# Tom94/practical-path-guiding

Hardware: NVIDIA H100
Metric: Msamples/sec (paths x bounces) (higher is better)
Workload: dtype f32

## Files before the change

### practical-path-guiding_b200/csrc/ppg_bounce.cuh

```cuda
#pragma once
#include "ppg_wavefront.cuh"

namespace ppg {

template <bool FIRST, int RECORD, bool NEE, bool SMEM, bool FULL>
__global__ void __launch_bounds__(SMEM ? PPG_BOUNCE_BLOCK : PPG_BOUNCE_BLOCK_HBM, SMEM ? PPG_MIN_BLOCKS : PPG_MIN_BLOCKS_HBM) bounce_kernel(const __grid_constant__ RenderParams P) {
    const SceneAccess<SMEM> sc(P.scene);
    sc.stage();
    const uint32_t nIn = FIRST ? P.nPaths : *P.liveIn;
    uint32_t raysLocal = 0, recLocal = 0, levelsLocal = 0;
    __shared__ uint32_t binStart[PPG_BINS + 1];
    const bool binned = !SMEM && P.order != nullptr;
    if (binned) {
        if (threadIdx.x == 0) { uint32_t acc = 0; for (uint32_t b = 0; b < PPG_BINS; ++b) { binStart[b] = acc; acc += P.binCount[b]; } binStart[PPG_BINS] = acc; }
        __syncthreads();
    }

    const uint32_t lane = threadIdx.x & 31u;
    uint32_t claimBase = 0, claimLeft = 0;
    for (;;) {
        if (claimLeft == 0) {
            if (lane == 0) claimBase = atomicAdd(P.work, 32u * PPG_CLAIM);
            claimBase = __shfl_sync(0xffffffffu, claimBase, 0);
            claimLeft = PPG_CLAIM;
        }
        if (claimBase >= nIn) break;
        uint32_t i = claimBase + lane;
        claimBase += 32u; --claimLeft;
        bool alive = i < nIn;
        if (binned && alive) {
            uint32_t b = 0;
            while (b + 1 < PPG_BINS && i >= binStart[b + 1]) ++b;
            i = __ldg(&P.order[(size_t) b * P.binStride + (i - binStart[b])]);
        }
        float3 o, d, thr, Li; float eta = 1.f, rrRecip = 1.f, mint, maxt;
        float prevWoPdf = 0.f; float3 prevRefN = f3(0, 0, 0); uint32_t prevSlot = 0;
        uint32_t pathId = 0, nVertices = 0, flags = 0;
        Pcg32 rng; rng.state = 0; rng.inc = 1;
        if (alive) {
            if (FIRST) {
                pathId = i;
                uint64_t sampleIndex;
                camera_ray(P, i, rng, sampleIndex, o, d, mint, maxt);
                thr = f3(1, 1, 1); Li = f3(0, 0, 0);
            } else {
                const float4 a = __ldcs(&P.in.s0[i]), b = __ldcs(&P.in.s1[i]), c = __ldcs(&P.in.s2[i]), e = __ldcs(&P.in.s3[i]), f = __ldcs(&P.in.s4[i]);
                o = f3(a.x, a.y, a.z); d = f3(a.w, b.x, b.y); thr = f3(b.z, b.w, c.x); eta = c.y; Li = f3(c.z, c.w, e.x);
                pathId = __float_as_uint(e.y);
                rng.state = ((uint64_t) __float_as_uint(e.w) << 32) | __float_as_uint(e.z);
                const uint64_t sampleIndex = ((uint64_t) __float_as_uint(f.y) << 32) | __float_as_uint(f.x);
                rng.inc = (sampleIndex << 1) | 1u;
                const uint32_t nf = __float_as_uint(f.z); nVertices = nf & 0xffu; flags = nf >> 8;
                rrRecip = f.w;
                if (NEE) { const float4 g5 = __ldcs(&P.in.s5[i]), g6 = __ldcs(&P.in.s6[i]); prevWoPdf = g5.x; prevRefN = f3(g5.y, g5.z, g5.w); prevSlot = __float_as_uint(g6.x); }
                mint = surface_ray_mint(o);
                maxt = __int_as_float(0x7f800000);
            }
        }
        bool wroteVertex = false, wroteNee = false, unscattered = FIRST;
        Hit hit; bool rayOk = false, found = false;
        if (alive) {
            ++raysLocal;
            rayOk = isfinite(o.x + o.y + o.z) && isfinite(d.x + d.y + d.z);
            if (!rayOk) atomicAdd(&P.counters[5], 1ull);
            if (!SMEM && P.hits) {
                const float4 hv = __ldcs(&P.hits[i]);
                const uint32_t w = __float_as_uint(hv.w);
                hit.t = hv.x; hit.u = hv.y; hit.v = hv.z; hit.tri = 0; hit.prim = w;
                found = rayOk && w != 0xFFFFFFFFu;
                if (found && !(w & PPG_SPHERE_BIT)) { hit.tri = w; hit.prim = __float_as_uint(sc.accel(3 * w + 2).z); }
                if (!found) { hit.t = __int_as_float(0x7f800000); hit.prim = 0xFFFFFFFFu; }
            } else
                found = rayOk && bvh_intersect<FULL>(sc, o, d, mint, maxt, hit);
        }
        __syncwarp();
        if (alive) {
            bool cont = found;
            if (FULL && !found && rayOk && P.scene.envW) {
                const bool viaNull = !FIRST && (flags & PPG_FLAG_NULL);
                const bool add = (FIRST || viaNull) ? ((FIRST || (flags & PPG_FLAG_UNSCATTERED)) && !P.hideEmitters) : true;
                if (add) {
                    float3 Lenv = thr * env_eval(P.scene, d);
                    if (NEE && !FIRST && !viaNull && P.doNee && !(prevSlot >> 31))
                        Lenv = Lenv * mi_weight(prevWoPdf, pdf_emitter_direct<FULL>(P.scene, PPG_ENV_EMITTER, o, prevRefN, d, f3(0, 0, 0), 0.f));
                    Li = Li + Lenv;
                }
                if (NEE && !FIRST && !viaNull && P.training && P.neeMode == 2 && ((prevSlot >> 30) & 1u)) {
                    const uint32_t ps = prevSlot & 0x3fffffffu;
                    float4 pv = P.prevSlab.v2[ps]; pv.x = Li.x; pv.y = Li.y; pv.z = Li.z; P.prevSlab.v2[ps] = pv;
                }
            }
            Its its;
            if (cont) {
                fill_its<FULL>(sc, hit, o, d, its);
                float3 Lhit = f3(0, 0, 0);
                const bool viaNull = FULL && !FIRST && (flags & PPG_FLAG_NULL);
                unscattered = FIRST || (FULL && (flags & PPG_FLAG_UNSCATTERED));
                if (FULL && viaNull) {
                    if (its.emitter >= 0 && unscattered && !P.hideEmitters && dot(its.shN, -d) > 0.f) {
                        const float4 r = sc.radiance(its.emitter);
                        Li = Li + thr * f3(r.x, r.y, r.z);
                    }
                } else if (FULL && !FIRST && its.emitter < 0 && bsdf_has_null(load_bsdf<FULL>(sc, its.bsdf))) {
                    int qEmitter; float3 qN; float qDist;
                    const float3 value = look_through(sc, o, d, its, hit.t, P.maxDepth - P.depth, qEmitter, qN, qDist);
                    if (!is_zero(value)) {
                        Lhit = thr * value;
                        if (NEE && P.doNee && !(prevSlot >> 31)) Lhit = Lhit * mi_weight(prevWoPdf, pdf_emitter_direct<FULL>(sc.g, qEmitter, o, prevRefN, d, qN, qDist));
                        Li = Li + Lhit;
                    }
                } else if (its.emitter >= 0 && (!FIRST || !P.hideEmitters)) {
                    if (dot(its.shN, -d) > 0.f) {
                        const float4 r = sc.radiance(its.emitter);
                        Lhit = thr * f3(r.x, r.y, r.z);
                        if (NEE && !FIRST && P.doNee && !(prevSlot >> 31)) {
                            const float emitterPdf = pdf_emitter_direct<FULL>(sc.g, its.emitter, o, prevRefN, d, its.shN, hit.t);
                            Lhit = Lhit * mi_weight(prevWoPdf, emitterPdf);
                        }
                        Li = Li + Lhit;
                    }
                }
                if (NEE && !FIRST && P.training && P.neeMode == 2 && ((prevSlot >> 30) & 1u)) {
                    const uint32_t ps = prevSlot & 0x3fffffffu;
                    float4 pv = P.prevSlab.v2[ps]; pv.x = Li.x; pv.y = Li.y; pv.z = Li.z; P.prevSlab.v2[ps] = pv;
                }
                thr = thr * rrRecip;
                if (flags & PPG_FLAG_DYING) cont = false;
                if (P.depth >= P.maxDepth && P.maxDepth != -1) cont = false;
            }
            if (cont) {
                const float wiDotGeoN = -dot(its.geoN, d);
                if (wiDotGeoN * its.wi.z < 0.f && P.strictNormals) cont = false;
            }
            if (cont) {
                Bsdf bsdf = load_bsdf<FULL>(sc, its.bsdf);
                const float3 n0 = its.shN;
                const bool bump = FULL && bsdf.bumpTex && !(hit.prim & PPG_SPHERE_BIT);
                if (FULL && (bsdf.reflTex | bsdf.bumpTex) && !(hit.prim & PPG_SPHERE_BIT)) apply_textures(sc, hit, d, its, bsdf);
                const bool smooth = bsdf_has_smooth(bsdf);
                int levels = 0; uint32_t leaf = 0; float4 la = make_float4(0, 0, 0, 0);
                if (smooth) {
                    leaf = stree_lookup(P.tree.snodes, P.tree.stable, P.tree.aabbMin, P.tree.extent, its.p, levels);
                    la = __ldg(&P.tree.leafA[leaf]);
                }
                float frac = P.fixedFraction;
                if (smooth && P.lossMode != 0) frac = logistic(la.z);
                float woPdf, bsdfPdf, dTreePdf, bsEta = 1.f; float3 wo, bsdfWeight; bool isDelta = false, isNull = false;
                float sx = rng.next1D(); const float sy = rng.next1D();
                if (!P.isBuilt || !smooth) {
                    bsdfWeight = bsdf_sample(bsdf, its.wi, sx, sy, wo, bsEta, isDelta, bsdfPdf, rng, isNull);
                    if (bump && !is_zero(bsdfWeight) && dot(its.toWorld(wo), n0) * wo.z <= 0.f) bsdfWeight = f3(0, 0, 0);
                    woPdf = bsdfPdf; dTreePdf = 0.f;
                } else {
                    const SampNode *tree = P.tree.samp + __float_as_uint(la.x);
                    const bool valid = __float_as_uint(la.w) & 1u;
                    float3 result; bool zero = false, deltaEarly = false;
                    if (sx < frac) {
                        sx /= frac;
                        result = bsdf_sample(bsdf, its.wi, sx, sy, wo, bsEta, isDelta, bsdfPdf, rng, isNull);
                        if (bump && !is_zero(result) && dot(its.toWorld(wo), n0) * wo.z <= 0.f) result = f3(0, 0, 0);
                        if (is_zero(result)) { woPdf = bsdfPdf = dTreePdf = 0.f; zero = true; }
                        else if (FULL && isDelta) { dTreePdf = 0.f; woPdf = bsdfPdf * frac; result = result * (1.0f / frac); deltaEarly = true; }
                        else result = result * bsdfPdf;
                    } else {
                        const float2 c2 = dtree_sample(tree, valid, rng);
                        const float3 dw = canonical_to_dir(c2);
                        wo = its.toLocal(dw);
                        result = (bump && dot(dw, n0) * wo.z <= 0.f) ? f3(0, 0, 0) : bsdf_eval(bsdf, its.wi, wo);
                    }
                    if (zero) bsdfWeight = f3(0, 0, 0);
                    else if (deltaEarly) bsdfWeight = result;
                    else {
                        bsdfPdf = (bump && dot(its.toWorld(wo), n0) * wo.z <= 0.f) ? 0.0f : bsdf_pdf(bsdf, its.wi, wo);
                        if (!isfinite(bsdfPdf)) { woPdf = 0.f; dTreePdf = 0.f; }
                        else {
                            dTreePdf = dtree_pdf(tree, valid, dir_to_canonical(its.toWorld(wo)));
                            woPdf = frac * bsdfPdf + (1.f - frac) * dTreePdf;
                        }
                        bsdfWeight = (woPdf == 0.f) ? f3(0, 0, 0) : result * (1.0f / woPdf);
                    }
                }
                const float3 refN = bsdf_has_transmission_or_backside(bsdf) ? f3(0, 0, 0) : n0;
                if (NEE && P.doNee && smooth) {
                    const float ex = rng.next1D(), ey = rng.next1D();
                    DirectSample ds; float dist;
                    if (sample_emitter_direct<FULL>(sc, its.p, refN, ex, ey, ds, dist)) {
                        const float smint = PPG_EPSILON * fmaxf(fmaxf(fabsf(its.p.x), fabsf(its.p.y)), fabsf(its.p.z));
                        Hit sh;
                        bool visible;
                        if (FULL) {
                            const float3 T = eval_transmittance(sc, its.p, ds.d, dist, P.maxDepth - P.depth - 1);
                            ds.value = ds.value * T; visible = !is_zero(ds.value);
                        } else visible = !bvh_intersect<FULL>(sc, its.p, ds.d, smint, dist * (1.f - PPG_SHADOW_EPSILON), sh);
                        if (visible) {
                            const float3 dl = its.toLocal(ds.d);
                            const float dlZ0 = bump ? dot(ds.d, n0) : dl.z;
                            if (!P.strictNormals || dot(its.geoN, ds.d) * dlZ0 > 0.f) {
                                const bool bumpReject = bump && dlZ0 * dl.z <= 0.f;
                                const float3 bsdfVal = bumpReject ? f3(0, 0, 0) : bsdf_eval(bsdf, its.wi, dl);
                                float nWoPdf = 0.f, nBsdfPdf = bumpReject ? 0.0f : bsdf_pdf(bsdf, its.wi, dl), nDTreePdf = 0.f;
                                if (!P.isBuilt) nWoPdf = nBsdfPdf;
                                else if (isfinite(nBsdfPdf)) {
                                    nDTreePdf = dtree_pdf(P.tree.samp + __float_as_uint(la.x), __float_as_uint(la.w) & 1u, dir_to_canonical(ds.d));
                                    nWoPdf = frac * nBsdfPdf + (1.f - frac) * nDTreePdf;
                                }
                                const float3 L = thr * (ds.value * bsdfVal) * mi_weight(ds.pdf, nWoPdf);
                                if (RECORD && P.neeMode != 2) {
                                    const float3 tv = thr * bsdfVal * (1.0f / ds.pdf);
                                    __stcs(&P.neeSlab.v0[i], make_float4(ds.d.x, ds.d.y, ds.d.z, ds.pdf));
                                    __stcs(&P.neeSlab.v1[i], make_float4(tv.x, tv.y, tv.z, __uint_as_float(leaf)));
                                    __stcs(&P.neeSlab.v2[i], make_float4(L.x, L.y, L.z, __uint_as_float(pathId | 0x40000000u)));
                                    __stcs(&P.neeSlab.v3[i], make_float4(bsdfVal.x, bsdfVal.y, bsdfVal.z, nBsdfPdf));
                                    __stcs(&P.neeSlab.v4[i], make_float4(its.p.x, its.p.y, its.p.z, nDTreePdf));
                                    __stcs(&P.neeSlab.v5[i], make_float4(__uint_as_float((uint32_t) (rng.inc >> 1)), __uint_as_float((uint32_t) (rng.inc >> 33)),
                                                                  __uint_as_float((uint32_t) levels | ((32u + (uint32_t) P.depth) << 8)), 0.f));
                                    wroteNee = true;
                                }
                                Li = Li + L;
                            }
                        }
                    }
                }
                if (is_zero(bsdfWeight)) cont = false;
                float3 woW = f3(0, 0, 0);
                if (cont) {
                    woW = its.toWorld(wo);
                    if (dot(its.geoN, woW) * (bump ? dot(woW, n0) : wo.z) <= 0.f && P.strictNormals) cont = false;
                }
                if (cont) {
                    o = its.p; d = woW;
                    thr = thr * bsdfWeight; eta *= bsEta;
                    if (RECORD && smooth && (!isDelta || P.lossMode != 0) && nVertices < PPG_MAX_VERTICES && (1.f / woPdf > 0.f)) {
                        __stcs(&P.slab.v0[i], make_float4(d.x, d.y, d.z, woPdf));
                        __stcs(&P.slab.v1[i], make_float4(thr.x, thr.y, thr.z, __uint_as_float(leaf)));
                        __stcs(&P.slab.v2[i], make_float4(Li.x, Li.y, Li.z, __uint_as_float(pathId | (isDelta ? 0x80000000u : 0u))));
                        if (RECORD == 2) {
                            const float3 bv = bsdfWeight * woPdf;
                            __stcs(&P.slab.v3[i], make_float4(bv.x, bv.y, bv.z, bsdfPdf));
                            __stcs(&P.slab.v4[i], make_float4(o.x, o.y, o.z, dTreePdf));
                            __stcs(&P.slab.v5[i], make_float4(__uint_as_float((uint32_t) (rng.inc >> 1)), __uint_as_float((uint32_t) (rng.inc >> 33)),
                                                       __uint_as_float((uint32_t) levels | (nVertices << 8)), 0.f));
                        }
                        wroteVertex = true; ++nVertices; ++recLocal; levelsLocal += levels;
                    }
                    if (NEE) { prevWoPdf = woPdf; prevRefN = refN; prevSlot = i | (isDelta ? 0x80000000u : 0u) | ((wroteVertex && !(FULL && isNull)) ? 0x40000000u : 0u); }
                    rrRecip = 1.f; flags = 0;
                    if (FULL && isNull) flags = PPG_FLAG_NULL | (unscattered ? PPG_FLAG_UNSCATTERED : 0u);
                    else if (P.depth >= P.rrDepth) {
                        float successProb = 1.0f;
                        if (smooth && !isDelta) {
                            if (!P.isBuilt) successProb = max3(thr) * eta * eta;
                            successProb = fmaxf(0.1f, fminf(successProb, 0.99f));
                        }
                        if (rng.next1D() >= successProb) flags |= PPG_FLAG_DYING;
                        else rrRecip = 1.0f / successProb;
                    }
                }
            }
            if (!cont) {
                __stcs(&P.liFinal[pathId], make_float4(Li.x, Li.y, Li.z, 1.f));
                alive = false;
            }
        }
        if (RECORD && i < nIn && !wroteVertex) __stcs(&P.slab.v2[i], make_float4(0.f, 0.f, 0.f, __uint_as_float(PPG_INVALID)));
        if (NEE && RECORD && P.neeMode != 2 && i < nIn && !wroteNee) __stcs(&P.neeSlab.v2[i], make_float4(0.f, 0.f, 0.f, __uint_as_float(PPG_INVALID)));
        const uint32_t slot = warp_compact(alive, P.liveOut);
        if (alive) {
            __stcs(&P.out.s0[slot], make_float4(o.x, o.y, o.z, d.x));
            __stcs(&P.out.s1[slot], make_float4(d.y, d.z, thr.x, thr.y));
            __stcs(&P.out.s2[slot], make_float4(thr.z, eta, Li.x, Li.y));
            __stcs(&P.out.s3[slot], make_float4(Li.z, __uint_as_float(pathId), __uint_as_float((uint32_t) rng.state), __uint_as_float((uint32_t) (rng.state >> 32))));
            __stcs(&P.out.s4[slot], make_float4(__uint_as_float((uint32_t) (rng.inc >> 1)), __uint_as_float((uint32_t) (rng.inc >> 33)),
                                         __uint_as_float(nVertices | (flags << 8)), rrRecip));
            if (NEE) {
                __stcs(&P.out.s5[slot], make_float4(prevWoPdf, prevRefN.x, prevRefN.y, prevRefN.z));
                __stcs(&P.out.s6[slot], make_float4(__uint_as_float(prevSlot), 0.f, 0.f, 0.f));
            }
        }
    }
    unsigned long long rays = raysLocal, rec = recLocal, lev = levelsLocal;
    for (int off = 16; off; off >>= 1) {
        rays += __shfl_xor_sync(0xffffffffu, rays, off);
        rec += __shfl_xor_sync(0xffffffffu, rec, off);
        lev += __shfl_xor_sync(0xffffffffu, lev, off);
    }
    if ((threadIdx.x & 31) == 0) {
        if (rays) atomicAdd(&P.counters[0], rays);
        if (rec) { atomicAdd(&P.counters[1], rec); atomicAdd(&P.counters[2], lev); }
    }
}

}
```

### practical-path-guiding_b200/csrc/ppg_device.cuh

```cuda
#pragma once
#include <cuda_runtime.h>
#include <cuda_fp16.h>
#include <stdint.h>
#include "ppg_scene_layout.h"

namespace ppg {

#define PPG_PI 3.14159265358979323846f
#define PPG_INV_PI 0.31830988618379067154f
#define PPG_EPSILON 1e-4f

__device__ __forceinline__ float3 f3(float x, float y, float z) { return make_float3(x, y, z); }
__device__ __forceinline__ float3 operator+(float3 a, float3 b) { return f3(a.x + b.x, a.y + b.y, a.z + b.z); }
__device__ __forceinline__ float3 operator-(float3 a, float3 b) { return f3(a.x - b.x, a.y - b.y, a.z - b.z); }
__device__ __forceinline__ float3 operator*(float3 a, float s) { return f3(a.x * s, a.y * s, a.z * s); }
__device__ __forceinline__ float3 operator*(float3 a, float3 b) { return f3(a.x * b.x, a.y * b.y, a.z * b.z); }
__device__ __forceinline__ float3 operator-(float3 a) { return f3(-a.x, -a.y, -a.z); }
__device__ __forceinline__ float dot(float3 a, float3 b) { return a.x * b.x + a.y * b.y + a.z * b.z; }
__device__ __forceinline__ float3 cross(float3 a, float3 b) { return f3(a.y * b.z - a.z * b.y, a.z * b.x - a.x * b.z, a.x * b.y - a.y * b.x); }
__device__ __forceinline__ float3 normalize(float3 a) { return a * (1.0f / sqrtf(dot(a, a))); }
__device__ __forceinline__ bool is_zero(float3 a) { return a.x == 0.f && a.y == 0.f && a.z == 0.f; }
__device__ __forceinline__ bool is_valid(float3 a) {
    return isfinite(a.x) && isfinite(a.y) && isfinite(a.z) && a.x >= 0.f && a.y >= 0.f && a.z >= 0.f;
}
// ... 33 lines not shown
__device__ __forceinline__ void seed_vertex_rng(Pcg32 &r, uint64_t seed, uint64_t sampleIndex, uint32_t ordinal) {
    r.seed(splitmix64((seed + 0x5851F42D4C957F2Dull) ^ splitmix64(sampleIndex * 64 + ordinal)), sampleIndex * 64 + ordinal);
}

#define PPG_ENV_EMITTER (-2)

struct Hit { float t, u, v; uint32_t tri; uint32_t prim; };

extern __shared__ float4 ppg_scene_smem[];
template <bool SMEM> struct SceneAccess {
    static constexpr bool kStaged = SMEM;
    const SceneView &g;
    uint32_t oGeom, oMeta, oBvh, oBsdf, oRadiance, oGroups;
    __device__ __forceinline__ SceneAccess(const SceneView &v) : g(v) {
        oGeom = 3 * v.nTris; oMeta = oGeom + 6 * v.nTris; oBvh = oMeta + v.nTris; oBsdf = oBvh + 2 * v.nBvhNodes;
        oRadiance = oBsdf + PPG_BSDF_F4 * v.nBsdfs; oGroups = oRadiance + v.nEmitters;
    }
    __device__ __forceinline__ float4 accel(uint32_t i) const { return SMEM ? ppg_scene_smem[i] : __ldg(&g.accel[i]); }
    __device__ __forceinline__ float4 geom(uint32_t i) const { return SMEM ? ppg_scene_smem[oGeom + i] : __ldg(&g.geom[i]); }
    __device__ __forceinline__ int4 meta(uint32_t i) const {
        if (SMEM) { const float4 m = ppg_scene_smem[oMeta + i]; return make_int4(__float_as_int(m.x), __float_as_int(m.y), __float_as_int(m.z), __float_as_int(m.w)); }
        return __ldg(&g.meta[i]);
    }
    __device__ __forceinline__ float4 bvh(uint32_t i) const { return SMEM ? ppg_scene_smem[oBvh + i] : __ldg(&g.bvh[i]); }
    __device__ __forceinline__ float4 bsdf(uint32_t i) const { return SMEM ? ppg_scene_smem[oBsdf + i] : __ldg(&g.bsdf[i]); }
    __device__ __forceinline__ float4 radiance(uint32_t i) const { return SMEM ? ppg_scene_smem[oRadiance + i] : __ldg(&g.radiance[i]); }
    __device__ __forceinline__ float4 groups(uint32_t i) const { return SMEM ? ppg_scene_smem[oGroups + i] : __ldg(&g.groups[i]); }
    __device__ __forceinline__ void stage() const {
        if (!SMEM) return;
        auto copy = [&](uint32_t off, const float4 *src, uint32_t n) { for (uint32_t i = threadIdx.x; i < n; i += blockDim.x) ppg_scene_smem[off + i] = src[i]; };
        copy(0, g.accel, 3 * g.nTris); copy(oGeom, g.geom, 6 * g.nTris); copy(oMeta, reinterpret_cast<const float4 *>(g.meta), g.nTris);
        copy(oBvh, g.bvh, 2 * g.nBvhNodes); copy(oBsdf, g.bsdf, PPG_BSDF_F4 * g.nBsdfs); copy(oRadiance, g.radiance, g.nEmitters); copy(oGroups, g.groups, 2 * g.nGroups);
        __syncthreads();
    }
};

__device__ __forceinline__ bool tri_intersect(const float4 A, const float4 B, const float4 C, float3 o, float3 d, float mint, float maxt,
                                              float &u, float &v, float &t) {
    const int k = __float_as_int(A.w);
    float o_u, o_v, o_k, d_u, d_v, d_k;
    if (k == 0) { o_u = o.y; o_v = o.z; o_k = o.x; d_u = d.y; d_v = d.z; d_k = d.x; }
    else if (k == 1) { o_u = o.z; o_v = o.x; o_k = o.y; d_u = d.z; d_v = d.x; d_k = d.y; }
    else if (k == 2) { o_u = o.x; o_v = o.y; o_k = o.z; d_u = d.x; d_v = d.y; d_k = d.z; }
    else return false;
    t = (A.z - o_u * A.x - o_v * A.y - o_k) / (d_u * A.x + d_v * A.y + d_k);
    if (!(t >= mint && t <= maxt)) return false;
    const float hu = o_u + t * d_u - B.x;
    const float hv = o_v + t * d_v - B.y;
    u = hv * B.z + hu * B.w;
    v = hu * C.x + hv * C.y;
    return u >= 0.f && v >= 0.f && u + v <= 1.0f;
}

template <class Acc>
__device__ __forceinline__ void tri_group_exact(const Acc &A_, uint32_t q, float o_u, float o_v, float o_k, float d_u, float d_v, float d_k,
                                                float mint, float maxt, Hit &hit) {
    const uint32_t fc = __float_as_uint(A_.groups(2 * q).w), last = (fc & 0xffffu) + (fc >> 16);
    for (uint32_t i = fc & 0xffffu; i < last; ++i) {
        const float4 A = A_.accel(3 * i), B = A_.accel(3 * i + 1), C = A_.accel(3 * i + 2);
        const float t = (A.z - o_u * A.x - o_v * A.y - o_k) / (d_u * A.x + d_v * A.y + d_k);
        if (t >= mint && t <= maxt) {
            const float hu = o_u + t * d_u - B.x, hv = o_v + t * d_v - B.y;
            const float u = hv * B.z + hu * B.w, v = hu * C.x + hv * C.y;
            if (u >= 0.f && v >= 0.f && u + v <= 1.0f) {
                const uint32_t prim = __float_as_uint(C.z);
                if (t < hit.t || (t == hit.t && prim < hit.prim)) { hit.t = t; hit.u = u; hit.v = v; hit.prim = prim; hit.tri = i; }
            }
        }
    }
}

__device__ __forceinline__ bool sphere_intersect(float4 cr, float3 ro, float3 rd, float mint, float maxt, float &t) {
    const double ox = (double) ro.x - (double) cr.x, oy = (double) ro.y - (double) cr.y, oz = (double) ro.z - (double) cr.z;
    const double dx = rd.x, dy = rd.y, dz = rd.z;
    const double A = __dadd_rn(__dadd_rn(__dmul_rn(dx, dx), __dmul_rn(dy, dy)), __dmul_rn(dz, dz));
    const double B = __dmul_rn(2.0, __dadd_rn(__dadd_rn(__dmul_rn(ox, dx), __dmul_rn(oy, dy)), __dmul_rn(oz, dz)));
    const double C = __dsub_rn(__dadd_rn(__dadd_rn(__dmul_rn(ox, ox), __dmul_rn(oy, oy)), __dmul_rn(oz, oz)), (double) (cr.w * cr.w));
    double nearT, farT;
    if (A == 0.0) { if (B != 0.0) nearT = farT = -C / B; else return false; }
    else {
        const double discrim = __dsub_rn(__dmul_rn(B, B), __dmul_rn(__dmul_rn(4.0, A), C));
        if (discrim < 0.0) return false;
        const double sqrtDiscrim = sqrt(discrim);
        const double temp = B < 0.0 ? __dmul_rn(-0.5, __dsub_rn(B, sqrtDiscrim)) : __dmul_rn(-0.5, __dadd_rn(B, sqrtDiscrim));
        nearT = temp / A; farT = C / temp;
        if (nearT > farT) { const double s = nearT; nearT = farT; farT = s; }
    }
    if (!(nearT <= (double) maxt && farT >= (double) mint)) return false;
    if (nearT < (double) mint) { if (farT > (double) maxt) return false; t = (float) farT; }
    else t = (float) nearT;
    return true;
}
__device__ __forceinline__ bool bvh_slab(float3 o, float3 inv, float mint, float tmax, const float4 n0, const float4 n1, float &tEntry) {
    float ta = (n0.x - o.x) * inv.x, tb = (n1.x - o.x) * inv.x; if (ta > tb) { const float s_ = ta; ta = tb; tb = s_; }
    float nearMax = fmaxf(__int_as_float(0xff800000), ta), farMin = fminf(__int_as_float(0x7f800000), tb);
    ta = (n0.y - o.y) * inv.y; tb = (n1.y - o.y) * inv.y; if (ta > tb) { const float s_ = ta; ta = tb; tb = s_; }
    nearMax = fmaxf(nearMax, ta); farMin = fminf(farMin, tb);
    ta = (n0.z - o.z) * inv.z; tb = (n1.z - o.z) * inv.z; if (ta > tb) { const float s_ = ta; ta = tb; tb = s_; }
    nearMax = fmaxf(nearMax, ta); farMin = fminf(farMin, tb);
    const float t0 = fmaxf(mint, nearMax * (nearMax > 0.f ? 1.0f - 1e-6f : 1.0f + 1e-6f)), t1 = fminf(tmax, farMin * (farMin > 0.f ? 1.0f + 1e-6f : 1.0f - 1e-6f));
    tEntry = t0;
    return t0 <= t1;
}
static __device__ __noinline__ Hit bvh_walk(const float4 *__restrict__ accel, const float4 *__restrict__ bvh, float3 o, float3 d, float mint, float maxt) {
    Hit hit; hit.t = __int_as_float(0x7f800000); hit.u = hit.v = 0.f; hit.prim = 0xFFFFFFFFu; hit.tri = 0;
    const float3 inv = f3(1.0f / d.x, 1.0f / d.y, 1.0f / d.z);
    auto slab = [&](const float4 n0, const float4 n1, float &tEntry) -> bool { return bvh_slab(o, inv, mint, fminf(maxt, hit.t), n0, n1, tEntry); };
    auto node = [&](uint32_t i) { return __ldg(&bvh[i]); };
    auto tri = [&](uint32_t i) { return __ldg(&accel[i]); };
    uint32_t stackN[PPG_BVH_STACK]; float stackT[PPG_BVH_STACK]; int sp = 0;
    uint32_t left, count;
    {
        const float4 r0 = node(0), r1 = node(1);
        float te;
        if (!slab(r0, r1, te)) return hit;
        left = __float_as_uint(r0.w); count = __float_as_uint(r1.w);
    }
    auto pop = [&]() -> bool {
        while (sp > 0) {
            --sp;
            if (stackT[sp] <= hit.t) { left = stackN[sp] & 0x0fffffffu; count = stackN[sp] >> 28; return true; }
        }
        return false;
    };
    bool done = false;
    for (;;) {
        while (count == 0u && !done) {
            const float4 a0 = node(2 * left), a1 = node(2 * left + 1), b0 = node(2 * left + 2), b1 = node(2 * left + 3);
            float ta, tb;
            const bool ha = slab(a0, a1, ta), hb = slab(b0, b1, tb);
            if (ha && hb) {
                const bool aFirst = ta <= tb;
                const float4 f0 = aFirst ? b0 : a0, f1 = aFirst ? b1 : a1, n0 = aFirst ? a0 : b0, n1 = aFirst ? a1 : b1;
                stackN[sp] = __float_as_uint(f0.w) | (__float_as_uint(f1.w) << 28); stackT[sp] = aFirst ? tb : ta; ++sp;
                left = __float_as_uint(n0.w); count = __float_as_uint(n1.w);
            } else if (ha) { left = __float_as_uint(a0.w); count = __float_as_uint(a1.w); }
            else if (hb) { left = __float_as_uint(b0.w); count = __float_as_uint(b1.w); }
            else done = !pop();
        }
        if (done) break;
        for (uint32_t i = left; i < left + count; ++i) {
            const float4 A = tri(3 * i), B = tri(3 * i + 1), C = tri(3 * i + 2);
            float u, v, t;
            if (tri_intersect(A, B, C, o, d, mint, maxt, u, v, t)) {
                const uint32_t prim = __float_as_uint(C.z);
                if (t < hit.t || (t == hit.t && prim < hit.prim)) { hit.t = t; hit.u = u; hit.v = v; hit.prim = prim; hit.tri = i; }
            }
        }
        if (!pop()) break;
    }
    return hit;
}
template <class Acc> __device__ __forceinline__ bool tri_scene_intersect(const Acc &A_, float3 o, float3 d, float mint, float maxt, Hit &hit);

template <bool SPHERES, class Acc>
__device__ __forceinline__ bool bvh_intersect(const Acc &A_, float3 o, float3 d, float mint, float maxt, Hit &hit) {
    bool found = tri_scene_intersect(A_, o, d, mint, maxt, hit);
    if (!SPHERES) return found;
    const SceneView &sc = A_.g;
    for (uint32_t k = 0; k < sc.nSpheres; ++k) {
        float t;
        if (sphere_intersect(__ldg(&sc.spheres[2 * k]), o, d, mint, maxt, t) && t < hit.t) { hit.t = t; hit.u = hit.v = 0.f; hit.prim = PPG_SPHERE_BIT | k; hit.tri = 0; found = true; }
    }
    return found;
}
template <class Acc>
__device__ __forceinline__ bool tri_scene_intersect(const Acc &A_, float3 o, float3 d, float mint, float maxt, Hit &hit) {
    const SceneView &sc = A_.g;
    hit.t = __int_as_float(0x7f800000); hit.prim = 0xFFFFFFFFu; hit.tri = 0;
    if (sc.nTris == 0u) return false;
    if (Acc::kStaged || sc.nGroups != 0u) {
        const float tlo = mint * (1.0f - 1e-4f), thi = maxt * (1.0f + 1e-4f);
        uint32_t cand = 0, nearQ = 0xFFFFFFFFu; float nearT = __int_as_float(0x7f800000);
#pragma unroll 1
        for (int g = 0; g < 3; ++g) {
            float o_u, o_v, o_k, d_u, d_v, d_k;
            if (g == 0) { o_u = o.y; o_v = o.z; o_k = o.x; d_u = d.y; d_v = d.z; d_k = d.x; }
            else if (g == 1) { o_u = o.z; o_v = o.x; o_k = o.y; d_u = d.z; d_v = d.x; d_k = d.y; }
            else { o_u = o.x; o_v = o.y; o_k = o.z; d_u = d.x; d_v = d.y; d_k = d.z; }
            const uint32_t end = sc.kBegin[g + 1];
#pragma unroll 1
            for (uint32_t q = sc.kBegin[g]; q < end; ++q) {
                const float4 G0 = A_.groups(2 * q);
                const float ta = __fdividef(G0.z - o_u * G0.x - o_v * G0.y - o_k, d_u * G0.x + d_v * G0.y + d_k);
                if (ta >= tlo && ta <= thi) {
                    const float4 G1 = A_.groups(2 * q + 1);
                    const float pu = o_u + ta * d_u, pv = o_v + ta * d_v;
                    if (pu >= G1.x && pv >= G1.y && pu <= G1.z && pv <= G1.w) {
                        cand |= 1u << q; if (ta < nearT) { nearT = ta; nearQ = q; }
                    }
                }
            }
        }
        if (nearQ != 0xFFFFFFFFu) {
            const uint32_t q = nearQ; cand &= ~(1u << q);
            const int k = (q >= sc.kBegin[1]) + (q >= sc.kBegin[2]);
            const float o_u = k == 0 ? o.y : (k == 1 ? o.z : o.x), o_v = k == 0 ? o.z : (k == 1 ? o.x : o.y), o_k = k == 0 ? o.x : (k == 1 ? o.y : o.z);
            const float d_u = k == 0 ? d.y : (k == 1 ? d.z : d.x), d_v = k == 0 ? d.z : (k == 1 ? d.x : d.y), d_k = k == 0 ? d.x : (k == 1 ? d.y : d.z);
            tri_group_exact(A_, q, o_u, o_v, o_k, d_u, d_v, d_k, mint, maxt, hit);
        }
        while (cand) {
            const uint32_t q = __ffs(cand) - 1; cand &= cand - 1u;
            const int k = (q >= sc.kBegin[1]) + (q >= sc.kBegin[2]);
            const float o_u = k == 0 ? o.y : (k == 1 ? o.z : o.x), o_v = k == 0 ? o.z : (k == 1 ? o.x : o.y), o_k = k == 0 ? o.x : (k == 1 ? o.y : o.z);
            const float d_u = k == 0 ? d.y : (k == 1 ? d.z : d.x), d_v = k == 0 ? d.z : (k == 1 ? d.x : d.y), d_k = k == 0 ? d.x : (k == 1 ? d.y : d.z);
            const float4 G0 = A_.groups(2 * q);
            const float ta = __fdividef(G0.z - o_u * G0.x - o_v * G0.y - o_k, d_u * G0.x + d_v * G0.y + d_k);
            if (ta <= hit.t * (1.0f + 1e-4f)) tri_group_exact(A_, q, o_u, o_v, o_k, d_u, d_v, d_k, mint, maxt, hit);
        }
        return hit.prim != 0xFFFFFFFFu;
    }
    hit = bvh_walk(sc.accel, sc.bvh, o, d, mint, maxt);
    return hit.prim != 0xFFFFFFFFu;
}

struct Its {
    float3 p, geoN, shN, shS, shT, wi;
    int bsdf, emitter;
    __device__ __forceinline__ float3 toLocal(float3 v) const { return f3(dot(v, shS), dot(v, shT), dot(v, shN)); }
    __device__ __forceinline__ float3 toWorld(float3 v) const { return shS * v.x + shT * v.y + shN * v.z; }
};

template <bool SPHERES, class Acc>
__device__ __forceinline__ void fill_its(const Acc &A_, const Hit &h, float3 o, float3 d, Its &its) {
    if (SPHERES && (h.prim & PPG_SPHERE_BIT)) {
        const uint32_t k = h.prim & ~PPG_SPHERE_BIT;
        const float4 cr = __ldg(&A_.g.spheres[2 * k]), mt = __ldg(&A_.g.spheres[2 * k + 1]);
        const float3 c = f3(cr.x, cr.y, cr.z);
        its.p = o + d * h.t;
        its.p = c + normalize(its.p - c) * cr.w;
        const float3 local = its.p - c;
        const float3 dpdu = f3(-local.y, local.x, 0.f) * (2.f * PPG_PI);
        its.geoN = normalize(its.p - c);
        if (__float_as_uint(mt.z)) its.geoN = its.geoN * -1.0f;
        its.shN = its.geoN;
        its.shS = normalize(dpdu - its.shN * dot(its.shN, dpdu));
        its.shT = cross(its.shN, its.shS);
        its.wi = its.toLocal(-d);
        its.bsdf = __float_as_int(mt.x); its.emitter = __float_as_int(mt.y);
        return;
    }
    const float4 g0 = A_.geom(6 * h.tri), g1 = A_.geom(6 * h.tri + 1), g2 = A_.geom(6 * h.tri + 2);
    const int4 m = A_.meta(h.tri);
    const float3 p0 = f3(g0.x, g0.y, g0.z), p1 = f3(g1.x, g1.y, g1.z), p2 = f3(g2.x, g2.y, g2.z);
    const float3 b = f3(1 - h.u - h.v, h.u, h.v);
    its.p = p0 * b.x + p1 * b.y + p2 * b.z;
    const float3 side1 = p1 - p0, side2 = p2 - p0;
    float3 faceN = cross(side1, side2);
    const float len = sqrtf(dot(faceN, faceN));
    if (!is_zero(faceN)) faceN = faceN * (1.0f / len);
    if (m.z & 1) {
        const float4 h0 = A_.geom(6 * h.tri + 3), h1 = A_.geom(6 * h.tri + 4), h2 = A_.geom(6 * h.tri + 5);
        const float3 n0 = f3(g0.w, h0.x, h0.y), n1 = f3(g1.w, h1.x, h1.y), n2 = f3(g2.w, h2.x, h2.y);
        its.shN = normalize(n0 * b.x + n1 * b.y + n2 * b.z);
        if (dot(faceN, its.shN) < 0.f) faceN = -faceN;
    } else its.shN = faceN;
    its.geoN = faceN;
    const float3 dpdu = side1;
    its.shS = normalize(dpdu - its.shN * dot(its.shN, dpdu));
    its.shT = cross(its.shN, its.shS);
    its.wi = its.toLocal(-d);
    its.bsdf = m.x; its.emitter = m.y;
}

__device__ __forceinline__ float3 square_to_cosine_hemisphere(float sx, float sy) {
    const float r1 = 2.0f * sx - 1.0f, r2 = 2.0f * sy - 1.0f;
    float phi, r;
    if (r1 == 0.f && r2 == 0.f) { r = phi = 0.f; }
    else if (r1 * r1 > r2 * r2) { r = r1; phi = (PPG_PI / 4.0f) * (r2 / r1); }
    else { r = r2; phi = (PPG_PI / 2.0f) - (r1 / r2) * (PPG_PI / 4.0f); }
    float s, c; sincosf_bounded(phi, &s, &c);
    const float px = r * c, py = r * s;
    float z = sqrtf(fmaxf(0.0f, 1.0f - px * px - py * py));
    if (z == 0.f) z = 1e-10f;
    return f3(px, py, z);
}
#define PPG_BSDF_TWOSIDED 1u
#define PPG_BSDF_T_DIFFUSE 0u
#define PPG_BSDF_T_DIELECTRIC 2u
#define PPG_BSDF_T_CONDUCTOR 3u
#define PPG_BSDF_T_ROUGHCONDUCTOR 4u
#define PPG_BSDF_T_ROUGHPLASTIC 5u
#define PPG_BSDF_T_ROUGHDIELECTRIC 6u
#define PPG_BSDF_T_PLASTIC 7u
#define PPG_BSDF_T_THINDIELECTRIC 8u
#define PPG_BSDF_NONLINEAR 2u
#define PPG_BSDF_MASK 4u
#define PPG_BSDF_BUMPMAP 8u
struct Bsdf { float3 refl, trans, etaRgb, k, specRefl, opacity; float eta, invEta, alpha, fdrInt, ssw, maskProb; uint32_t type, flags; int distr; const float *lut;
              uint32_t reflTex, bumpTex; };
template <bool FULL, class Acc>
__device__ __forceinline__ Bsdf load_bsdf(const Acc &A_, int idx) {
    const float4 a = A_.bsdf(PPG_BSDF_F4 * idx);
    Bsdf b; b.refl = f3(a.x, a.y, a.z);
    const uint32_t tf = __float_as_uint(a.w); b.type = FULL ? (tf & 0xffu) : PPG_BSDF_T_DIFFUSE; b.flags = tf >> 8;
    b.trans = b.etaRgb = b.k = b.specRefl = f3(0, 0, 0); b.eta = b.invEta = 1.f; b.alpha = 0.1f; b.distr = 1; b.fdrInt = b.ssw = 0.f; b.lut = nullptr;
    b.opacity = f3(1, 1, 1); b.maskProb = 1.f; b.reflTex = b.bumpTex = 0u;
    if (FULL) { const float4 w = A_.bsdf(PPG_BSDF_F4 * idx + 5); b.reflTex = __float_as_uint(w.z); b.bumpTex = (b.flags & PPG_BSDF_BUMPMAP) ? __float_as_uint(w.w) : 0u; }
    if (FULL && (b.flags & PPG_BSDF_MASK)) { const float4 m = A_.bsdf(PPG_BSDF_F4 * idx + 6); b.opacity = f3(m.x, m.y, m.z); b.maskProb = m.w; }
    if (!FULL) b.flags &= PPG_BSDF_TWOSIDED;
    if (FULL && b.type != PPG_BSDF_T_DIFFUSE) {
        const float4 t = A_.bsdf(PPG_BSDF_F4 * idx + 1), e = A_.bsdf(PPG_BSDF_F4 * idx + 2), k = A_.bsdf(PPG_BSDF_F4 * idx + 3);
        b.trans = f3(t.x, t.y, t.z); b.eta = t.w; b.etaRgb = f3(e.x, e.y, e.z); b.invEta = e.w; b.k = f3(k.x, k.y, k.z);
        b.alpha = fabsf(k.w); b.distr = k.w < 0.f ? 0 : 1;
        if (b.type == PPG_BSDF_T_ROUGHPLASTIC || b.type == PPG_BSDF_T_PLASTIC) {
            const float4 s = A_.bsdf(PPG_BSDF_F4 * idx + 4), w = A_.bsdf(PPG_BSDF_F4 * idx + 5);
            b.specRefl = f3(s.x, s.y, s.z); b.fdrInt = s.w; b.ssw = w.x; b.lut = A_.g.bsdfTables + (size_t) __float_as_uint(w.y) * PPG_BSDF_LUT;
        }
    }
    return b;
}
__device__ __forceinline__ bool bsdf_has_smooth(const Bsdf &b) { return b.type == PPG_BSDF_T_DIFFUSE || b.type == PPG_BSDF_T_ROUGHCONDUCTOR || b.type == PPG_BSDF_T_ROUGHPLASTIC || b.type == PPG_BSDF_T_ROUGHDIELECTRIC || b.type == PPG_BSDF_T_PLASTIC; }
__device__ __forceinline__ bool bsdf_has_transmission_or_backside(const Bsdf &b) { return (b.flags & (PPG_BSDF_TWOSIDED | PPG_BSDF_MASK)) || b.type == PPG_BSDF_T_DIELECTRIC || b.type == PPG_BSDF_T_ROUGHDIELECTRIC || b.type == PPG_BSDF_T_THINDIELECTRIC; }
__device__ __forceinline__ bool bsdf_has_null(const Bsdf &b) { return b.type == PPG_BSDF_T_THINDIELECTRIC || (b.flags & PPG_BSDF_MASK); }

__device__ __forceinline__ float fresnel_dielectric_ext(float cosThetaI_, float &cosThetaT_, float eta) {
    if (eta == 1.f) { cosThetaT_ = -cosThetaI_; return 0.0f; }
    const float scale = (cosThetaI_ > 0.f) ? 1.f / eta : eta, cosThetaTSqr = 1.f - (1.f - cosThetaI_ * cosThetaI_) * (scale * scale);
    if (cosThetaTSqr <= 0.0f) { cosThetaT_ = 0.0f; return 1.0f; }
    const float cosThetaI = fabsf(cosThetaI_), cosThetaT = sqrtf(cosThetaTSqr);
    const float Rs = (cosThetaI - eta * cosThetaT) / (cosThetaI + eta * cosThetaT);
    const float Rp = (eta * cosThetaI - cosThetaT) / (eta * cosThetaI + cosThetaT);
    cosThetaT_ = (cosThetaI_ > 0.f) ? -cosThetaT : cosThetaT;
    return 0.5f * (Rs * Rs + Rp * Rp);
}
__device__ __forceinline__ float fresnel_conductor_exact(float cosThetaI, float eta, float k) {
    const float cosThetaI2 = cosThetaI * cosThetaI, sinThetaI2 = 1.f - cosThetaI2, sinThetaI4 = sinThetaI2 * sinThetaI2;
    const float temp1 = eta * eta - k * k - sinThetaI2;
    const float a2pb2 = sqrtf(fmaxf(0.0f, temp1 * temp1 + k * k * eta * eta * 4.f));
    const float a = sqrtf(fmaxf(0.0f, (a2pb2 + temp1) * 0.5f));
    const float term1 = a2pb2 + cosThetaI2, term2 = a * (2.f * cosThetaI);
    const float Rs2 = (term1 - term2) / (term1 + term2);
    const float term3 = a2pb2 * cosThetaI2 + sinThetaI4, term4 = term2 * sinThetaI2;
    const float Rp2 = Rs2 * (term3 - term4) / (term3 + term4);
    return 0.5f * (Rp2 + Rs2);
}
__device__ __forceinline__ float mts_erfinv(float x) {
    float w = -logf((1.0f - x) * (1.0f + x)), p;
    if (w < 5.0f) {
        w = w - 2.5f; p = 2.81022636e-08f; p = 3.43273939e-07f + p * w; p = -3.5233877e-06f + p * w; p = -4.39150654e-06f + p * w;
// ... 952 lines not shown
```

### practical-path-guiding_b200/csrc/ppg_wavefront.cuh

```cuda
#pragma once
#include "ppg_device.cuh"

namespace ppg {

#ifndef PPG_BLOCK
#define PPG_BLOCK 256
#endif
#ifndef PPG_BOUNCE_BLOCK
#define PPG_BOUNCE_BLOCK 1024
#endif
#ifndef PPG_BOUNCE_BLOCK_HBM
#define PPG_BOUNCE_BLOCK_HBM 256
#endif
#ifndef PPG_MIN_BLOCKS
#define PPG_MIN_BLOCKS 1
#endif
#ifndef PPG_CLAIM
#define PPG_CLAIM 1u
#endif
#ifndef PPG_MIN_BLOCKS_HBM
#define PPG_MIN_BLOCKS_HBM 4
#endif
#define PPG_MAX_VERTICES 32
#define PPG_INVALID 0xFFFFFFFFu

struct PathState {
    float4 *s0;
    float4 *s1;
    float4 *s2;
    float4 *s3;
    float4 *s4;
    float4 *s5;
    float4 *s6;
};
#define PPG_FLAG_NULL 2u
#define PPG_FLAG_UNSCATTERED 4u
#define PPG_FLAG_DYING 1u

struct VertexSlab {
    float4 *v0;
    float4 *v1;
    float4 *v2;
    float4 *v3;
    float4 *v4;
    float4 *v5;
};

struct RenderParams {
    SceneView scene; Camera cam; TreeView tree;
    PathState in, out;
    VertexSlab slab;
    float4 *liFinal;
    const uint32_t *pixelMap;
    const uint32_t *liveIn; uint32_t *liveOut;
    uint32_t *work;
    unsigned long long *counters;
    uint32_t nPaths;
    uint32_t nLocalPixels, spp;
    uint64_t passBase;
    uint64_t seed;
    int depth;
    int maxDepth, rrDepth;
    int strictNormals, hideEmitters;
    int isBuilt;
    int lossMode;
    float fixedFraction;
    uint32_t sceneSmemBytes;
    int neeMode, doNee;
    int training;
    VertexSlab neeSlab;
    VertexSlab prevSlab;
    float4 *hits;
    uint32_t *traceWork;
    uint32_t *order;
    uint32_t *binCount;
    uint32_t binStride;
};
#define PPG_BINS 16u

__device__ __forceinline__ void camera_ray(const RenderParams &P, uint32_t i, Pcg32 &rng, uint64_t &sampleIndex, float3 &o, float3 &d, float &mint, float &maxt) {
    const uint32_t perPass = P.nLocalPixels * P.spp;
    const uint32_t passInBatch = i / perPass, rem = i - passInBatch * perPass;
    const uint32_t lp = rem / P.spp, s = rem - lp * P.spp;
    const uint32_t xy = __ldg(&P.pixelMap[lp]);
    const uint32_t x = xy & 0xffffu, y = xy >> 16;
    sampleIndex = (((P.passBase + passInBatch) * (uint64_t) P.cam.H + y) * (uint64_t) P.cam.W + x) * P.spp + s;
    seed_path_rng(rng, P.seed, sampleIndex);
    const float jx = rng.next1D(), jy = rng.next1D();
    const float sx = ((float) x + jx) * (1.0f / (float) P.cam.W), sy = ((float) y + jy) * (1.0f / (float) P.cam.H);
    const float3 nearP = f3((1.0f - 2.0f * sx) * P.cam.tanX, (1.0f - 2.0f * sy) * P.cam.tanY, 1.0f);
    const float3 dl = normalize(nearP);
    const float invZ = 1.0f / dl.z;
    mint = P.cam.nearClip * invZ; maxt = P.cam.farClip * invZ;
    o = P.cam.o;
    d = P.cam.left * dl.x + P.cam.up * dl.y + P.cam.dir * dl.z;
}
__device__ __forceinline__ float surface_ray_mint(float3 o) { return PPG_EPSILON * fmaxf(fmaxf(fmaxf(fabsf(o.x), fabsf(o.y)), fabsf(o.z)), PPG_EPSILON); }

__device__ __forceinline__ uint32_t warp_compact(bool alive, uint32_t *counter) {
    const unsigned ballot = __ballot_sync(0xffffffffu, alive);
    const int lane = threadIdx.x & 31;
    uint32_t base = 0;
    if (lane == 0 && ballot) base = atomicAdd(counter, (uint32_t) __popc(ballot));
    base = __shfl_sync(0xffffffffu, base, 0);
    return base + __popc(ballot & ((1u << lane) - 1u));
}

struct BounceLaunch { cudaStream_t stream; int grid; int record; int nee; int first; };
void ppg_launch_bounce_00(const RenderParams &P, const BounceLaunch &L); void ppg_launch_bounce_01(const RenderParams &P, const BounceLaunch &L);
void ppg_launch_bounce_10(const RenderParams &P, const BounceLaunch &L); void ppg_launch_bounce_11(const RenderParams &P, const BounceLaunch &L);
void ppg_launch_trace(const RenderParams &P, cudaStream_t stream, int grid, bool first, bool spheres);
int ppg_trace_occupancy();
int ppg_bounce_occupancy_00(size_t smem); int ppg_bounce_occupancy_01(size_t smem); int ppg_bounce_occupancy_10(size_t smem); int ppg_bounce_occupancy_11(size_t smem);

}
```

Measured before the change: 4889.

## Defer path-state loads past traversal, warp-aggregate stats, fuse group filter math

In the shared-memory, non-first, non-NEE bounce kernel, only origin and direction are loaded before BVH traversal. The remaining path state is prefetched to L2 and loaded after traversal, so fewer registers stay live across the traversal loop. Per-thread ray and record counters are replaced by per-warp ballot/reduce accumulation in shared memory. The group-filter intersection test is rewritten with FMAs. The extra ballots and shared-memory updates add work on every iteration, and the deferred loads may stall after traversal if the prefetched lines have been evicted from L2.

```diff
diff --git a/practical-path-guiding_b200/csrc/ppg_bounce.cuh b/practical-path-guiding_b200/csrc/ppg_bounce.cuh
--- a/practical-path-guiding_b200/csrc/ppg_bounce.cuh
+++ b/practical-path-guiding_b200/csrc/ppg_bounce.cuh
@@ -5,9 +5,14 @@
 
 template <bool FIRST, int RECORD, bool NEE, bool SMEM, bool FULL>
 __global__ void __launch_bounds__(SMEM ? PPG_BOUNCE_BLOCK : PPG_BOUNCE_BLOCK_HBM, SMEM ? PPG_MIN_BLOCKS : PPG_MIN_BLOCKS_HBM) bounce_kernel(const __grid_constant__ RenderParams P) {
+    constexpr bool DEFER = SMEM && !FIRST && !NEE;
     const SceneAccess<SMEM> sc(P.scene);
     sc.stage();
     const uint32_t nIn = FIRST ? P.nPaths : *P.liveIn;
+    constexpr bool WARP_STATS = SMEM;
+    __shared__ uint32_t warpRays[WARP_STATS ? 32 : 1], warpRec[WARP_STATS ? 32 : 1], warpLevels[WARP_STATS ? 32 : 1];
+    const uint32_t warp = WARP_STATS ? threadIdx.x >> 5 : 0;
+    if (WARP_STATS && (threadIdx.x & 31u) == 0) { warpRays[warp] = 0; warpRec[warp] = 0; warpLevels[warp] = 0; }
     uint32_t raysLocal = 0, recLocal = 0, levelsLocal = 0;
     __shared__ uint32_t binStart[PPG_BINS + 1];
     const bool binned = !SMEM && P.order != nullptr;
@@ -43,6 +48,12 @@
                 uint64_t sampleIndex;
                 camera_ray(P, i, rng, sampleIndex, o, d, mint, maxt);
                 thr = f3(1, 1, 1); Li = f3(0, 0, 0);
+            } else if (DEFER) {
+                const float4 a = __ldcs(&P.in.s0[i]); const float2 b = __ldcs(reinterpret_cast<const float2 *>(P.in.s1) + 2 * i);
+                o = f3(a.x, a.y, a.z); d = f3(a.w, b.x, b.y);
+                prefetch_l2(&P.in.s2[i]); prefetch_l2(&P.in.s3[i]); prefetch_l2(&P.in.s4[i]);
+                mint = surface_ray_mint(o);
+                maxt = __int_as_float(0x7f800000);
             } else {
                 const float4 a = __ldcs(&P.in.s0[i]), b = __ldcs(&P.in.s1[i]), c = __ldcs(&P.in.s2[i]), e = __ldcs(&P.in.s3[i]), f = __ldcs(&P.in.s4[i]);
                 o = f3(a.x, a.y, a.z); d = f3(a.w, b.x, b.y); thr = f3(b.z, b.w, c.x); eta = c.y; Li = f3(c.z, c.w, e.x);
@@ -58,9 +69,10 @@
             }
         }
         bool wroteVertex = false, wroteNee = false, unscattered = FIRST;
+        uint32_t recLevels = 0;
         Hit hit; bool rayOk = false, found = false;
         if (alive) {
-            ++raysLocal;
+            if (!WARP_STATS) ++raysLocal;
             rayOk = isfinite(o.x + o.y + o.z) && isfinite(d.x + d.y + d.z);
             if (!rayOk) atomicAdd(&P.counters[5], 1ull);
             if (!SMEM && P.hits) {
@@ -74,6 +86,17 @@
                 found = rayOk && bvh_intersect<FULL>(sc, o, d, mint, maxt, hit);
         }
         __syncwarp();
+        if (DEFER && alive) {
+            const float2 b = __ldcs(reinterpret_cast<const float2 *>(P.in.s1) + 2 * i + 1);
+            const float4 c = __ldcs(&P.in.s2[i]), e = __ldcs(&P.in.s3[i]), f = __ldcs(&P.in.s4[i]);
+            thr = f3(b.x, b.y, c.x); eta = c.y; Li = f3(c.z, c.w, e.x);
+            pathId = __float_as_uint(e.y);
+            rng.state = ((uint64_t) __float_as_uint(e.w) << 32) | __float_as_uint(e.z);
+            const uint64_t sampleIndex = ((uint64_t) __float_as_uint(f.y) << 32) | __float_as_uint(f.x);
+            rng.inc = (sampleIndex << 1) | 1u;
+            const uint32_t nf = __float_as_uint(f.z); nVertices = nf & 0xffu; flags = nf >> 8;
+            rrRecip = f.w;
+        }
         if (alive) {
             bool cont = found;
             if (FULL && !found && rayOk && P.scene.envW) {
@@ -241,7 +264,8 @@
                             __stcs(&P.slab.v5[i], make_float4(__uint_as_float((uint32_t) (rng.inc >> 1)), __uint_as_float((uint32_t) (rng.inc >> 33)),
                                                        __uint_as_float((uint32_t) levels | (nVertices << 8)), 0.f));
                         }
-                        wroteVertex = true; ++nVertices; ++recLocal; levelsLocal += levels;
+                        wroteVertex = true; ++nVertices;
+                        if (WARP_STATS) recLevels = (uint32_t) levels; else { ++recLocal; levelsLocal += levels; }
                     }
                     if (NEE) { prevWoPdf = woPdf; prevRefN = refN; prevSlot = i | (isDelta ? 0x80000000u : 0u) | ((wroteVertex && !(FULL && isNull)) ? 0x40000000u : 0u); }
                     rrRecip = 1.f; flags = 0;
@@ -264,6 +288,11 @@
         }
         if (RECORD && i < nIn && !wroteVertex) __stcs(&P.slab.v2[i], make_float4(0.f, 0.f, 0.f, __uint_as_float(PPG_INVALID)));
         if (NEE && RECORD && P.neeMode != 2 && i < nIn && !wroteNee) __stcs(&P.neeSlab.v2[i], make_float4(0.f, 0.f, 0.f, __uint_as_float(PPG_INVALID)));
+        if (WARP_STATS) {
+            const uint32_t rays = __popc(__ballot_sync(0xffffffffu, i < nIn));
+            const uint32_t rec = RECORD ? __popc(__ballot_sync(0xffffffffu, wroteVertex)) : 0u, lev = RECORD ? __reduce_add_sync(0xffffffffu, recLevels) : 0u;
+            if (lane == 0) { warpRays[warp] += rays; if (RECORD) { warpRec[warp] += rec; warpLevels[warp] += lev; } }
+        }
         const uint32_t slot = warp_compact(alive, P.liveOut);
         if (alive) {
             __stcs(&P.out.s0[slot], make_float4(o.x, o.y, o.z, d.x));
@@ -279,12 +308,14 @@
         }
     }
     unsigned long long rays = raysLocal, rec = recLocal, lev = levelsLocal;
-    for (int off = 16; off; off >>= 1) {
-        rays += __shfl_xor_sync(0xffffffffu, rays, off);
-        rec += __shfl_xor_sync(0xffffffffu, rec, off);
-        lev += __shfl_xor_sync(0xffffffffu, lev, off);
-    }
-    if ((threadIdx.x & 31) == 0) {
+    if (WARP_STATS) { rays = warpRays[warp]; rec = warpRec[warp]; lev = warpLevels[warp]; }
+    else
+        for (int off = 16; off; off >>= 1) {
+            rays += __shfl_xor_sync(0xffffffffu, rays, off);
+            rec += __shfl_xor_sync(0xffffffffu, rec, off);
+            lev += __shfl_xor_sync(0xffffffffu, lev, off);
+        }
+    if (lane == 0) {
         if (rays) atomicAdd(&P.counters[0], rays);
         if (rec) { atomicAdd(&P.counters[1], rec); atomicAdd(&P.counters[2], lev); }
     }
diff --git a/practical-path-guiding_b200/csrc/ppg_device.cuh b/practical-path-guiding_b200/csrc/ppg_device.cuh
--- a/practical-path-guiding_b200/csrc/ppg_device.cuh
+++ b/practical-path-guiding_b200/csrc/ppg_device.cuh
@@ -209,6 +209,9 @@
     return hit;
 }
 template <class Acc> __device__ __forceinline__ bool tri_scene_intersect(const Acc &A_, float3 o, float3 d, float mint, float maxt, Hit &hit);
+__device__ __forceinline__ float group_filter_t(float4 G0, float o_u, float o_v, float o_k, float d_u, float d_v, float d_k) {
+    return __fdividef(fmaf(-o_v, G0.y, fmaf(-o_u, G0.x, G0.z)) - o_k, fmaf(d_v, G0.y, fmaf(d_u, G0.x, d_k)));
+}
 
 template <bool SPHERES, class Acc>
 __device__ __forceinline__ bool bvh_intersect(const Acc &A_, float3 o, float3 d, float mint, float maxt, Hit &hit) {
@@ -239,10 +242,10 @@
 #pragma unroll 1
             for (uint32_t q = sc.kBegin[g]; q < end; ++q) {
                 const float4 G0 = A_.groups(2 * q);
-                const float ta = __fdividef(G0.z - o_u * G0.x - o_v * G0.y - o_k, d_u * G0.x + d_v * G0.y + d_k);
+                const float ta = group_filter_t(G0, o_u, o_v, o_k, d_u, d_v, d_k);
                 if (ta >= tlo && ta <= thi) {
                     const float4 G1 = A_.groups(2 * q + 1);
-                    const float pu = o_u + ta * d_u, pv = o_v + ta * d_v;
+                    const float pu = fmaf(ta, d_u, o_u), pv = fmaf(ta, d_v, o_v);
                     if (pu >= G1.x && pv >= G1.y && pu <= G1.z && pv <= G1.w) {
                         cand |= 1u << q; if (ta < nearT) { nearT = ta; nearQ = q; }
                     }
diff --git a/practical-path-guiding_b200/csrc/ppg_wavefront.cuh b/practical-path-guiding_b200/csrc/ppg_wavefront.cuh
--- a/practical-path-guiding_b200/csrc/ppg_wavefront.cuh
+++ b/practical-path-guiding_b200/csrc/ppg_wavefront.cuh
@@ -95,6 +95,7 @@
     o = P.cam.o;
     d = P.cam.left * dl.x + P.cam.up * dl.y + P.cam.dir * dl.z;
 }
+__device__ __forceinline__ void prefetch_l2(const void *p) { asm volatile("prefetch.global.L2 [%0];" :: "l"(p)); }
 __device__ __forceinline__ float surface_ray_mint(float3 o) { return PPG_EPSILON * fmaxf(fmaxf(fmaxf(fabsf(o.x), fabsf(o.y)), fabsf(o.z)), PPG_EPSILON); }
 
 __device__ __forceinline__ uint32_t warp_compact(bool alive, uint32_t *counter) {
```

New measurement: 5068 (median of 6 runs). +3.7%, better.
